# francescoalemanno/KissABC.jl

Hardware: AMD Instinct MI355X
Metric: walker proposal+cost evals/sec at N=65536 walkers, D=8 (higher is better)
Workload: dtype f64

## Files before the change

kissabc.jl_amd/csrc/ais_inst.hip:

```cpp
#define KABC_FMA_C_VGPR
#include "ais_small_kernel.hpp"

#ifndef KABC_INST_COST
#error "compile with -DKABC_INST_COST=<cost id>"
#endif

namespace kabc {

template <int D, int COST, int PC, int PK>
static void launch_half(const AisArgs& a, hipStream_t s, unsigned nchains) {
    const unsigned grid = (unsigned)((a.rows_owned + kBatch - 1) / kBatch);
    if (grid == 0) return;
    hipLaunchKernelGGL((ais_half_kernel<D, COST, PC, PK>), dim3(grid, nchains), dim3(kAisBlock), 0, s, a);
}

#ifndef KABC_INST_DLO
#define KABC_INST_DLO 1
#endif
#ifndef KABC_INST_DHI
#define KABC_INST_DHI KABC_MAX_DIM
#endif
#ifndef KABC_INST_SUFFIX
#define KABC_INST_SUFFIX
#endif
#ifndef KABC_INST_PCSEL
#define KABC_INST_PCSEL 0
#endif
template <int COST, int D, int PCX>
static AisLaunchFn pick() {
    constexpr bool is_normal = (PCX % kPriorClasses) == kPriorNormal;
    constexpr bool pc_ok = KABC_INST_PCSEL == 0 || (KABC_INST_PCSEL == 1) == is_normal;
    if constexpr (pc_ok && D >= KABC_INST_DLO && D <= KABC_INST_DHI && cost_dim_ok_c(COST, D))
        return &launch_half<D, COST, PCX % kPriorClasses, PCX / kPriorClasses + 1>;
    else return nullptr;
}

template <int COST, int PCX, int... Ds>
static AisLaunchFn row(int D, std::integer_sequence<int, Ds...>) {
    AisLaunchFn f[] = {pick<COST, Ds + 1, PCX>()...};
    return (D >= 1 && D <= (int)sizeof...(Ds)) ? f[D - 1] : nullptr;
}

template <int COST, int... PCXs>
static AisLaunchFn table(int D, int pcx, std::integer_sequence<int, PCXs...>) {
    using Dims = std::make_integer_sequence<int, KABC_MAX_DIM>;
    AisLaunchFn r = nullptr;
    ((pcx == PCXs ? (void)(r = row<COST, PCXs>(D, Dims{})) : (void)0), ...);
    return r;
}

template <int COST, int D, int PCX>
static AisSmallLaunchFn pick_small() {
    constexpr int pc = PCX % kPriorClasses;
    constexpr bool is_normal = pc == kPriorNormal;
    constexpr bool pc_ok = KABC_INST_PCSEL == 0 || (KABC_INST_PCSEL == 1) == is_normal;
    if constexpr (pc_ok && pc != kPriorSimple && D >= KABC_INST_DLO &&
                  D <= KABC_INST_DHI && cost_dim_ok_c(COST, D))
        return &launch_ais_small<D, COST, pc, PCX / kPriorClasses + 1>;
    else return nullptr;
}
template <int COST, int PCX, int... Ds>
static AisSmallLaunchFn row_small(int D, std::integer_sequence<int, Ds...>) {
    AisSmallLaunchFn f[] = {pick_small<COST, Ds + 1, PCX>()...};
    return (D >= 1 && D <= (int)sizeof...(Ds)) ? f[D - 1] : nullptr;
}
template <int COST, int... PCXs>
static AisSmallLaunchFn table_small(int D, int pcx, std::integer_sequence<int, PCXs...>) {
    using Dims = std::make_integer_sequence<int, KABC_MAX_DIM>;
    AisSmallLaunchFn r = nullptr;
    ((pcx == PCXs ? (void)(r = row_small<COST, PCXs>(D, Dims{})) : (void)0), ...);
    return r;
}

#define KABC_CAT2(a, b) a##b
#define KABC_CAT(a, b) KABC_CAT2(a, b)
AisLaunchFn KABC_CAT(KABC_CAT(find_ais_kernel_cost_, KABC_INST_COST), KABC_INST_SUFFIX)(int D, int pcx) {
    return table<KABC_INST_COST>(D, pcx, std::make_integer_sequence<int, kAisVariants>{});
}

AisSmallLaunchFn KABC_CAT(KABC_CAT(find_ais_small_kernel_cost_, KABC_INST_COST), KABC_INST_SUFFIX)(int D, int pcx) {
    return table_small<KABC_INST_COST>(D, pcx, std::make_integer_sequence<int, kAisVariants>{});
}

}
```

kissabc.jl_amd/csrc/ais_kernels.hpp:

```cpp
#pragma once

#include "kabc_device.hpp"
#ifndef __HIPCC_RTC__
#include "launcher.hpp"
#endif

namespace kabc {

struct AisArgs {
    double* x_act;
    const double* x_comp;
    double* lp;
    double* ll;
    double* trace;
    int32_t* dbg;
    DevCounters* counters;
    unsigned long long* slots;
    const double* cost_params;
    const double* cost_data;
    int64_t cost_ndata;
    int64_t row_first;
    int64_t rows_owned;
    int64_t n_comp;
    uint64_t seed;
// ... 39 lines not shown
    double eps;
    unsigned long long retry_budget;
    PriorSet prior;
    kabc_prior_t raw[KABC_MAX_DIM];
    const uint64_t* seeds;
    unsigned long long* chain_retries;
    int64_t stride_act, stride_own;
    int64_t params_stride, data_stride;
};

constexpr int kInitBlock = 64;

constexpr int kAisBlock = 256;
constexpr int kBatch = 64;
constexpr int kChunk = 3;

template <int D>
struct RecGeom {
    static constexpr int NB = (D + 2) / 2;
    static constexpr int NZ = (D + 2 > 4) ? (D + 2) : 4;
};

template <int Q>
struct SubStepIx {
    static constexpr int value = Q;
};

template <int D, int CH>
struct RecBuf {
    uint32_t mva[CH][kBatch];
// ... 327 lines not shown
        if (lane < n_active) {
            const int64_t s = (int64_t)(t - A.t0);
#pragma unroll
            for (int j = 0; j < W; ++j) aux[j][lane] = A.aux[(s * W + j) * A.rows_owned + r0 + lane];
        }
        return;
    }
    kabc_cost_rng_t rng = {A.seed, t, w_base + (uint32_t)lane, KABC_DOM_AIS_COST, 0u, 0u, nullptr,
                           logtab};
    double a[W];
    kabc_cost_prepare(COST, A.cost_params, A.cost_data, A.cost_ndata, &rng, a);
#pragma unroll
    for (int j = 0; j < W; ++j) aux[j][lane] = a[j];
}

template <int D, int COST, int PC, int PK>
__global__ void __launch_bounds__(kAisBlock) __attribute__((amdgpu_waves_per_eu(2, 2)))
ais_half_kernel(const AisArgs A0) {
    AisArgs A = A0;
    if (A0.seeds) {
        const int64_t c = (int64_t)blockIdx.y;
        A.seed = A0.seeds[c];
        A.x_act += c * A0.stride_act;
        A.x_comp += c * A0.stride_comp;
        A.lp += c * A0.stride_own;
        A.ll += c * A0.stride_own;
        if (A0.trace) A.trace += c * A0.stride_trace;
        if (A0.aux) A.aux += c * A0.stride_aux;
        A.cost_params += c * A0.params_stride;
        A.cost_data += c * A0.data_stride;
    }
    __shared__ ChunkRec<D> rec[2];
    __shared__ uint8_t listB[kChunk][kBatch];

    __shared__ PriorDev sprior[D];
    __shared__ double sbox_lo[D], sbox_hi[D];
    constexpr bool kGaussBox = PC == kPriorSimple || PC == kPriorNormal;
    __shared__ __attribute__((aligned(16))) double sgb[kGaussBox ? D : 1][8];
    __shared__ __attribute__((aligned(16))) double slogtab[KABC_MATH_TAB_WORDS];
    constexpr int kNbTabs = (PC == kPriorGeneral) ? kNbTabsGeneral : 0;
    __shared__ double snb[kNbTabs > 0 ? (kNbTabs + 1) * kNbEntries : 1];
    constexpr int kAuxW = cost_aux_c(COST);
    __shared__ double saux[2][kChunk][kAuxW > 0 ? kAuxW : 1][kBatch];
    constexpr int kPre = ais_pre_blocks(COST, D);
    __shared__ double spre[2][kChunk][kPre > 0 ? 2 * kPre : 1][kBatch];

    const int wave = __builtin_amdgcn_readfirstlane(threadIdx.x >> 6), lane = threadIdx.x & (kWave - 1);
    const int64_t r0 = (int64_t)blockIdx.x * kBatch;
    const int64_t rem = A.rows_owned - r0;
    const int n_active = rem >= kBatch ? kBatch : (int)rem;
    const uint32_t w_base = A.id_base + (uint32_t)(A.row_first + r0);
    const int nchunks = (A.nt + kChunk - 1) / kChunk;
    const bool tprobe = (KABL & 128) && A.dbg;
    unsigned long long t_begin = 0, t_bar = 0;
    if (tprobe) t_begin = __builtin_amdgcn_s_memtime();
#define KABC_TIMED_BARRIER()                                              \
    do {                                                                  \
        if (tprobe) {                                                     \
            const unsigned long long tb_ = __builtin_amdgcn_s_memtime(); \
            __syncthreads();                                              \
            t_bar += __builtin_amdgcn_s_memtime() - tb_;                  \
        } else {                                                          \
            __syncthreads();                                              \
        }                                                                 \
    } while (0)

    auto comp_row = [&](uint32_t idx) -> const double* {
        return reinterpret_cast<const double*>(reinterpret_cast<const char*>(A.x_comp) +
                                               (size_t)(idx * (uint32_t)(D * sizeof(double))));
    };
    const bool active = (wave == 0) && (lane < n_active);
    const int64_t r = r0 + lane;
    const int64_t row = A.row_first + r;
    double x[D];
    double lp = 0.0, ll = 0.0;
    unsigned int n_eval = 0, n_acc = 0;
    int err = 0;
    if (active) {
        load_row<D>(A.x_act + row * D, x);
        lp = A.lp[r];
        ll = A.ll[r];
        if (!ld_valid(PK, lp, ll)) err = 2;
    }

    static_assert(KABC_MATH_TAB_WORDS == 2 * kAisBlock, "two table words per thread");
    const double tab0 = kabc_log_tab[threadIdx.x], tab1 = kabc_log_tab[threadIdx.x + kAisBlock];
    if (threadIdx.x < D * (int)(sizeof(PriorDev) / 8))
        reinterpret_cast<double*>(sprior)[threadIdx.x] =
            reinterpret_cast<const double*>(A.prior)[threadIdx.x];
    if (threadIdx.x < D) {
        sbox_lo[threadIdx.x] = A.prior[threadIdx.x].p[0];
        sbox_hi[threadIdx.x] = A.prior[threadIdx.x].p[1];
    }
    uint32_t dmask = 0, gmask = 0;
    for (int k = 0; k < D; ++k) {
        dmask |= (A.prior[k].discrete ? 1u : 0u) << k;
        gmask |= (gaussbox_is_gauss(A.prior[k].kind) ? 1u : 0u) << k;
    }
    if constexpr (kGaussBox) {
        if (threadIdx.x < D) gaussbox_stage(sgb[threadIdx.x], A.prior[threadIdx.x]);
    }
    const GaussBoxPrior gbox = {sgb, gmask, dmask};
    constexpr bool kBoxRegs = (PC == kPriorBox) && D <= 8;
    double blo[kBoxRegs ? D : 1], bhi[kBoxRegs ? D : 1];
    const BoxPrior box = {kBoxRegs ? blo : sbox_lo, kBoxRegs ? bhi : sbox_hi, dmask, A.box_lp};

    kabc_u128_t pro01[2] = {};
    if (wave > 0 && wave - 1 < A.nt && lane < n_active) {
        const uint32_t w = w_base + (uint32_t)lane;
        const uint64_t t = A.t0 + (uint64_t)(wave - 1);
        pro01[0] = kabc_stream_block(A.seed, w, t, 0u, KABC_DOM_AIS_MOVE);
        pro01[1] = kabc_stream_block(A.seed, w, t, 1u, KABC_DOM_AIS_MOVE);
    }
    slogtab[threadIdx.x] = tab0;
    slogtab[threadIdx.x + kAisBlock] = tab1;
#ifdef KABC_MODEL_SPEC
    [[maybe_unused]] const bool nb_on = kNbTabs > 0;
#else
    [[maybe_unused]] const bool nb_on = kNbTabs > 0 && A.nt >= 8;
#endif
    if constexpr (kNbTabs > 0) {
        static_assert(kNbEntries == kAisBlock, "one table entry per thread");
        int slot = 0;
        bool has_nb = false;
        for (int k = 0; k < D; ++k) {
            if (A.prior[k].kind == KABC_PRIOR_NEGBINOMIAL) {
                has_nb = true;
                if (nb_on && slot < kNbTabs) {
                    snb[slot * kNbEntries + threadIdx.x] =
                        kabc_lgamma_t((double)threadIdx.x + A.prior[k].p[0], kabc_log_tab);
                    ++slot;
                }
            }
        }
        if (has_nb) snb[kNbLg1Block * kNbEntries + threadIdx.x] = kabc_lgamma1_tab[threadIdx.x];
    }
    KABC_TIMED_BARRIER();
    if constexpr (kNbTabs > 0) {
        if (threadIdx.x < D && sprior[threadIdx.x].kind == KABC_PRIOR_NEGBINOMIAL) {
            int slot = 0;
            for (int k = 0; k < (int)threadIdx.x; ++k)
                slot += (sprior[k].kind == KABC_PRIOR_NEGBINOMIAL) ? 1 : 0;
            sprior[threadIdx.x].p[2] = (nb_on && slot < kNbTabs) ? (double)slot : -1.0;
        }
    }
    if constexpr (kBoxRegs) {
#pragma unroll
        for (int k = 0; k < D; ++k) {
            blo[k] = sbox_lo[k];
            bhi[k] = sbox_hi[k];
        }
    }

    uint64_t seed_v = A.seed;
    asm volatile("" : "+v"(seed_v));
    constexpr bool kLate = D > kLateFrom;
    double r0a[D], r0b[D], r1a[kLate ? 1 : D], r1b[kLate ? 1 : D];
    const bool pro_rows = !(KABL & 5);
    if (wave > 0) {
        const int si = wave - 1;
        if (si < A.nt && !(KABL & 4)) {
            produce_substep<D>(A, seed_v, rec[0], si, A.t0 + (uint64_t)si, w_base, n_active, listB[si],
                               lane, slogtab, pro01, [] { __syncthreads(); });
            if constexpr (kAuxW > 0)
                prepare_cost_aux<COST, kAuxW>(A, A.t0 + (uint64_t)si, w_base, lane, saux[0][si],
                                              slogtab, r0, n_active);
            if constexpr (kPre > 0)
                produce_cost_normals<kPre>(seed_v, A.t0 + (uint64_t)si, w_base, lane, spre[0][si], slogtab);
        } else {
            __syncthreads();
        }
    } else {
        __syncthreads();
#ifndef KABC_NO_XCHUNK_PREFETCH
        if (active && pro_rows) {
            load_row<D>(comp_row(rec[0].mva[0][lane] & 0x3fffffffu), r0a);
            load_row<D>(comp_row(rec[0].bb[0][lane]), r0b);
        }
#endif
    }
    KABC_TIMED_BARRIER();

    if (wave > 0) {
#pragma unroll 1
        for (int c = 0; c < nchunks; ++c) {
            const int s0 = c * kChunk;
            const int si = wave - 1;
            const int s = s0 + kChunk + si;
            if (s < A.nt && !(KABL & 2)) {
                produce_substep<D>(A, seed_v, rec[(c + 1) & 1], si, A.t0 + (uint64_t)s, w_base, n_active,
                                   listB[si], lane, slogtab);
                if constexpr (kAuxW > 0)
                    prepare_cost_aux<COST, kAuxW>(A, A.t0 + (uint64_t)s, w_base, lane,
                                                  saux[(c + 1) & 1][si], slogtab, r0, n_active);
                if constexpr (kPre > 0)
                    produce_cost_normals<kPre>(seed_v, A.t0 + (uint64_t)s, w_base, lane,
                                               spre[(c + 1) & 1][si], slogtab);
            }
            KABC_TIMED_BARRIER();
        }
    } else {
#ifndef KABC_NO_REG_PARAMS
        constexpr int kRP = cost_reg_params(COST, D);
        double cpar[kRP > 0 ? kRP : 1];
#pragma unroll
        for (int k = 0; k < kRP; ++k) {
            cpar[k] = A.cost_params[k];
            asm volatile("" : "+v"(cpar[k]));
        }
        const double* const cparams = kRP > 0 ? cpar : A.cost_params;
#else
        const double* const cparams = A.cost_params;
#endif
        const bool dbg_on = __builtin_amdgcn_readfirstlane(A.dbg != nullptr ? 1 : 0) != 0;
#pragma unroll 1
        for (int c = 0; c < nchunks; ++c) {
            const int s0 = c * kChunk;
            if (active && !(KABL & 1)) {
                const ChunkRec<D>& R = rec[(KABL & 2) ? 0 : (c & 1)];
                const int ns = (A.nt - s0 < kChunk) ? (A.nt - s0) : kChunk;
#ifndef KABC_NO_XCHUNK_PREFETCH
                if (c > 0 || !pro_rows)
#endif
                {
                    load_row<D>(comp_row(R.mva[0][lane] & 0x3fffffffu), r0a);
                    load_row<D>(comp_row(R.bb[0][lane]), r0b);
                }
                auto substep = [&](auto SI, const double (&pa)[D], const double (&pb)[D],
                                   double (&na)[D], double (&nb)[D]) __attribute__((always_inline)) {
                    constexpr int si = decltype(SI)::value;
                    const uint64_t t = A.t0 + (uint64_t)(s0 + si);
                    constexpr int sq = si + 1 < kChunk ? si + 1 : si;
                    const uint32_t mva = R.mva[si][lane];
                    uint32_t mvan = R.mva[sq][lane], bn = R.bb[sq][lane];
                    if (si + 1 >= ns) {
                        mvan = mva;
                        bn = R.bb[si][lane];
                    }
                    const double logu = R.logu[si][lane];
                    double zs[D + 1];
#pragma unroll
                    for (int j = 0; j < D + 1; ++j) zs[j] = R.zs[si][j][lane];
                    if constexpr (!kLate) {
                        load_row<D>(comp_row(mvan & 0x3fffffffu), na);
                        load_row<D>(comp_row(bn), nb);
                    }
                    __builtin_amdgcn_sched_barrier(0);
// ... 21 lines not shown
                            const double Wk = (pa[k] - pb[k]) * gamma;
                            const double sk = kabc_fabs(pa[k] - pb[k]) + kabc_fabs(x[k] - pb[k]) +
                                              kabc_fabs(xa[k]);
                            const double Tk = kabc_div_rc(gamma * sk, 300.0, 1.0 / 300.0) * zs[1 + k];
                            y[k] = x[k] + Wk + Tk;
                        }
                    }
                    __builtin_amdgcn_sched_barrier(0);
                    if constexpr (kLate) {
                        load_row<D>(comp_row(mvan & 0x3fffffffu), na);
                        load_row<D>(comp_row(bn), nb);
                    }
                    kabc_cost_rng_t rng = {A.seed, t, w_base + (uint32_t)lane, KABC_DOM_AIS_COST, 0u,
                                           0u, nullptr, slogtab};
                    if constexpr (kAuxW > 0) {
                        rng.aux = &saux[(KABL & 2) ? 0 : (c & 1)][si][0][lane];
                        rng.aux_stride = kBatch;
                    }
                    if constexpr (kPre > 0) {
                        rng.pre = &spre[(KABL & 2) ? 0 : (c & 1)][si][0][lane];
                        rng.pre_n = (uint32_t)kPre;
                        rng.pre_stride = (uint32_t)kBatch;
                    }
                    double nlp, nll;
                    bool ev;
                    loglike<D, COST, PC>(sprior, box, gbox, PK, A.eps, A.reps, y, cparams,
                                         A.cost_data, A.cost_ndata, &rng, nlp, nll, ev, slogtab,
                                         kNbTabs > 0 ? snb : nullptr);
                    __builtin_amdgcn_sched_barrier(0);
                    n_eval += ev ? 1u : 0u;
                    const bool valid = ev && ld_valid(PK, nlp, nll);
                    const double e = -logu;
                    bool acc;
                    if (PK == KABC_POSTERIOR_KERNELIZED) {
                        const double lW = corr + (nlp + nll) - (lp + ll);
// ... 14 lines not shown
                        ll = nll;
                        n_acc += 1u;
                    }
#pragma unroll
                    for (int k = 0; k < D; ++k) asm volatile("" : "+v"(x[k]));
                    if (dbg_on) {
                        int32_t* d = A.dbg + (r * A.dbg_nt + (A.dbg_s0 + s0 + si)) * 6;
                        d[0] = (int32_t)move;
                        d[1] = acc ? 1 : 0;
                        d[2] = (int32_t)(mva & 0x3fffffffu);
                        d[3] = move >= 2u ? (int32_t)R.bb[si][lane] : -1;
                        d[4] = move == 3u ? (int32_t)R.cc[si][lane] : -1;
                        d[5] = ev ? 1 : 0;
                    }
                };
                static_assert(kChunk == 3, "the consumer spells out kChunk sub-steps");
                if constexpr (kLate) {
                    substep(SubStepIx<0>{}, r0a, r0b, r0a, r0b);
                    if (ns > 1) substep(SubStepIx<1>{}, r0a, r0b, r0a, r0b);
                    if (ns > 2) substep(SubStepIx<2>{}, r0a, r0b, r0a, r0b);
                } else {
                    substep(SubStepIx<0>{}, r0a, r0b, r1a, r1b);
                    if (ns > 1) substep(SubStepIx<1>{}, r1a, r1b, r0a, r0b);
                    if (ns > 2) substep(SubStepIx<2>{}, r0a, r0b, r1a, r1b);
                }
            }
            KABC_TIMED_BARRIER();
        }
    }

    if (tprobe && lane == 0) {
        const unsigned long long t_end = __builtin_amdgcn_s_memtime();
        int32_t* d = A.dbg + (r0 * A.nt) * 6 + 8 + wave * 2;
        d[0] = (int32_t)(t_end - t_begin);
        d[1] = (int32_t)t_bar;
    }
    if ((KABL & 64) && A.dbg && lane == 0) {
        uint32_t hw;
        asm volatile("s_getreg_b32 %0, hwreg(HW_REG_HW_ID)" : "=s"(hw));
        A.dbg[(r0 * A.nt) * 6 + wave] = (int32_t)hw;
    }
    if (wave == 0) {
        if (active) {
            store_row<D>(A.x_act + row * D, x);
            A.lp[r] = lp;
            A.ll[r] = ll;
            if (A.trace) {
                double xp[D];
#pragma unroll
                for (int k = 0; k < D; ++k)
                    xp[k] = (sprior[k].discrete && PK != KABC_POSTERIOR_COMMON)
                                ? kabc_rint(x[k]) : x[k];
                store_row<D>(A.trace + r * D, xp);
            }
        }
        const unsigned long long se = wave_total_u32(n_eval);
        const unsigned long long sa = wave_total_u32(n_acc);
        if (lane == 0) {
            unsigned long long* sl =
                A.slots + (size_t)((blockIdx.x + blockIdx.y * gridDim.x) & (kCounterSlots - 1)) * 8;
            atomicAdd(&sl[0], (unsigned long long)n_active * (unsigned long long)A.nt);
            atomicAdd(&sl[1], se);
            atomicAdd(&sl[2], sa);
        }
        if (err) atomicMax(&A.counters->error, err);
    }
}

template <int D>
__global__ void __launch_bounds__(kInitBlock) ais_init_kernel(const InitArgs A) {
    const int64_t r = (int64_t)blockIdx.x * kInitBlock + threadIdx.x;
    if (r >= A.rows_owned) return;
    const int64_t row = A.row_first + r;
    const uint32_t w = A.id_base + (uint32_t)row;
    const int64_t chain = (int64_t)blockIdx.y;
    const uint64_t seed = A.seeds ? A.seeds[chain] : A.seed;
    unsigned long long* retries = A.seeds ? A.chain_retries + chain : &A.counters->retries;
    double* x_act = A.x_act + (A.seeds ? chain * A.stride_act : 0);
    double* lp_out = A.lp + (A.seeds ? chain * A.stride_own : 0);
    double* ll_out = A.ll + (A.seeds ? chain * A.stride_own : 0);
    const double* cparams = A.cost_params + (A.seeds ? chain * A.params_stride : 0);
// ... 44 lines not shown
    lp_out[r] = lp;
    ll_out[r] = ll;
}

#ifndef __HIPCC_RTC__
using AisLaunchFn = void (*)(const AisArgs&, hipStream_t, unsigned nchains);
using AisLaunch = Launcher<AisArgs, unsigned>;
using AisInitLaunch = Launcher<InitArgs, unsigned>;
inline dim3 ais_half_geom(const AisArgs& a, unsigned nchains) {
    return dim3((unsigned)((a.rows_owned + kBatch - 1) / kBatch), nchains);
}
inline dim3 ais_init_geom(const InitArgs& a, unsigned nchains) {
    return dim3((unsigned)((a.rows_owned + kInitBlock - 1) / kInitBlock), nchains);
}
AisLaunch find_ais_kernel(int cost_id, int D, int pcx);
constexpr int kAisVariants = 3 * kPriorClasses;
struct ModelUnit;
bool launch_ais_init(int D, const InitArgs& a, hipStream_t s, unsigned nchains, ModelUnit* unit);

#endif

}
```

kissabc.jl_amd/csrc/capi_ais.hip:

```cpp
#include <chrono>
#include <condition_variable>
#include <cstdio>
#include <cstdlib>
#include <mutex>
#include <thread>
#include <type_traits>
#include <vector>

#include "ais_aux_kernels.hpp"
#include "ais_dyn_kernels.hpp"
#include "ais_dyn_small_kernel.hpp"
#include "ais_small_kernel.hpp"
#include "host_common.hpp"
#include "plugin_registry.hpp"

namespace kabc {

#define KABC_DECL_COST(id)                                                \
    AisLaunchFn find_ais_kernel_cost_##id(int D, int pc);                 \
    AisLaunchFn find_ais_kernel_cost_##id##_nrm(int D, int pc);           \
    AisLaunchFn find_ais_kernel_cost_##id##_hi(int D, int pc);            \
    AisSmallLaunchFn find_ais_small_kernel_cost_##id(int D, int pc);      \
    AisSmallLaunchFn find_ais_small_kernel_cost_##id##_nrm(int D, int pc); \
    AisSmallLaunchFn find_ais_small_kernel_cost_##id##_hi(int D, int pc);
KABC_DECL_COST(1)
KABC_DECL_COST(2)
KABC_DECL_COST(3)
KABC_DECL_COST(4)
KABC_DECL_COST(5)
KABC_DECL_COST(6)
KABC_DECL_COST(7)
KABC_DECL_COST(8)
KABC_DECL_COST(9)
KABC_DECL_COST(10)
KABC_DECL_COST(11)

// ... 12 lines not shown
        case 3: return ais_inst_pick(D, pc, find_ais_kernel_cost_3, find_ais_kernel_cost_3_nrm, find_ais_kernel_cost_3_hi);
        case 4: return ais_inst_pick(D, pc, find_ais_kernel_cost_4, find_ais_kernel_cost_4_nrm, find_ais_kernel_cost_4_hi);
        case 5: return ais_inst_pick(D, pc, find_ais_kernel_cost_5, find_ais_kernel_cost_5_nrm, find_ais_kernel_cost_5_hi);
        case 6: return ais_inst_pick(D, pc, find_ais_kernel_cost_6, find_ais_kernel_cost_6_nrm, find_ais_kernel_cost_6_hi);
        case 7: return ais_inst_pick(D, pc, find_ais_kernel_cost_7, find_ais_kernel_cost_7_nrm, find_ais_kernel_cost_7_hi);
        case 8: return ais_inst_pick(D, pc, find_ais_kernel_cost_8, find_ais_kernel_cost_8_nrm, find_ais_kernel_cost_8_hi);
        case 9: return ais_inst_pick(D, pc, find_ais_kernel_cost_9, find_ais_kernel_cost_9_nrm, find_ais_kernel_cost_9_hi);
        case 10: return ais_inst_pick(D, pc, find_ais_kernel_cost_10, find_ais_kernel_cost_10_nrm, find_ais_kernel_cost_10_hi);
        case 11: return ais_inst_pick(D, pc, find_ais_kernel_cost_11, find_ais_kernel_cost_11_nrm, find_ais_kernel_cost_11_hi);
        default: {
            const PluginKernel k = plugin_kernel(find_plugin(cost_id), kPfAis, D, pc);
            if (k.host) return AisLaunch((AisLaunchFn)k.host);
            if (k.mod) return AisLaunch(k.mod, &ais_half_geom, (unsigned)kAisBlock);
            return nullptr;
        }
    }
}

static AisSmallLaunchFn ais_small_pick(int D, int pc, AisSmallLaunchFn (*lo)(int, int), AisSmallLaunchFn (*nrm)(int, int),
                                       AisSmallLaunchFn (*hi)(int, int)) {
    if (D > kAisInstSplit) return hi(D, pc);
    return (pc % kPriorClasses) == kPriorNormal ? nrm(D, pc) : lo(D, pc);
}
AisSmallLaunch find_ais_small_kernel(int cost_id, int D, int pc) {
#define KABC_SMALL_CASE(id) \
    case id: return AisSmallLaunch(ais_small_pick(D, pc, find_ais_small_kernel_cost_##id, find_ais_small_kernel_cost_##id##_nrm, find_ais_small_kernel_cost_##id##_hi));
    switch (cost_id) {
        KABC_SMALL_CASE(1)
        KABC_SMALL_CASE(2)
        KABC_SMALL_CASE(3)
// ... 81 lines not shown
    double* d_scratch = nullptr;
    int32_t nchains = 1;
    uint64_t* d_seeds = nullptr;
    unsigned long long* d_chain_retries = nullptr;
    uint32_t id_base[2] = {};
    double* d_half[2] = {};
    bool own_halves = false;
    double* d_lp[2] = {};
    double* d_ll[2] = {};
    DevCounters* d_counters = nullptr;
    unsigned long long* d_slots = nullptr;
    PriorDev* d_prior = nullptr;
    uint64_t seed = 0, t = 0;
    int32_t rank = 0, world = 1;
    AisLaunch launch;
    int32_t pc = 0;
    bool small_ok = false;
    AisSmallLaunch small;
    int32_t small_pcx = 0;
    AisDynSmallLaunchFn dsmall = nullptr;
    AisDynSmallPlan dplan;
    double* d_strace = nullptr;
    size_t strace_cap = 0;
    ModelUnit* unit = nullptr;
    int32_t spec_state = KABC_SPEC_NONE;
    int32_t spec_variant = 0;
    int64_t launches = 0;
    int64_t spec_switch_at = -1;
    std::chrono::steady_clock::time_point spec_next_poll;
    double box_lp = 0.0;
// ... 110 lines not shown
    AisLaunch fn;
    const int pk_off = kPriorClasses * (h->posterior - 1);
    if (h->unit) {
        int st = KABC_SPEC_NONE;
        PluginKernel uk;
        if (track || unit_required(h->unit)) uk = unit_kernel(h->unit, kPfAis, h->D, h->spec_variant, &st);
        if (uk.mod) fn = AisLaunch(uk.mod, &ais_half_geom, (unsigned)kAisBlock);
        if (track) h->spec_state = st;
        if (!fn && unit_required(h->unit)) return KABC_ERR_DEVICE;
    }
    if (!fn) {
        int pc = h->pc;
        if (const char* e = std::getenv("KABC_PREBUILT_CLASS"))
            if (e[0] == 'g' && pc != kPriorBox) pc = kPriorGeneral;
        fn = find_ais_kernel(h->cost_id, h->D, pc + pk_off);
        if (!fn && h->pc == kPriorNormal)
            fn = find_ais_kernel(h->cost_id, h->D, kPriorSimple + pk_off);
    }
    if (!fn) {
        if (!get_error()[0]) set_error("no gfx950 kernel instantiated for cost id %d, D = %d", h->cost_id, h->D);
        return KABC_ERR_UNSUPPORTED;
    }
    h->launch = fn;
    return KABC_OK;
}

static kabc_status_t ais_validate(kabc_ctx_t* ctx, const kabc_model_t* m, kabc_ais_t** out, int64_t n_total,
                                  int32_t rank, int32_t world, const kabc_comm_t* comm, int32_t nchains,
                                  std::vector<kabc_prior_t>& resolved, kabc_model_t& mres) {
    if (!ctx || !m || !out || !m->prior) {
// ... 661 lines not shown
static void timing_release(kabc_ais_t* h) {
    for (hipEvent_t e : h->ev) (void)hipEventDestroy(e);
    h->ev.clear();
    for (const kabc_ais::XT& x : h->xt) xt_release(x, h->xk);
    h->xt.clear();
}

static void ais_poll_spec(kabc_ais_t* h) {
    const auto now = std::chrono::steady_clock::now();
    if (now < h->spec_next_poll) return;
    h->spec_next_poll = now + std::chrono::milliseconds(2);
    int st = KABC_SPEC_NONE;
    const PluginKernel k = unit_kernel(h->unit, h->small_ok ? kPfAisSmall : kPfAis, h->D, h->spec_variant, &st);
    if (st == KABC_SPEC_ACTIVE && k.mod) {
        if (h->small_ok) h->small = AisSmallLaunch(k.mod, &ais_small_geom, (unsigned)kAisSmallBlock);
        else h->launch = AisLaunch(k.mod, &ais_half_geom, (unsigned)kAisBlock);
        h->spec_state = KABC_SPEC_ACTIVE;
        h->spec_switch_at = h->launches;
    } else if (st == KABC_SPEC_FAILED) {
        h->spec_state = KABC_SPEC_FAILED;
    }
}

static kabc_status_t launch_half_seg(kabc_ais_t* h, int32_t half, const kabc_ais::Seg& sg,
                                     int32_t ntransitions, double* dev_trace_rows) {
    if (sg.count == 0) return KABC_OK;
    hipStream_t s = h->ctx->stream;
    if (h->spec_state == KABC_SPEC_PENDING && !h->small_ok) ais_poll_spec(h);
    if (!h->launch && !h->dyn)
        if (kabc_status_t st = ais_resolve_half(h)) return st;
    if (h->dyn && h->nchains > 1) {
        set_error("a handle of %d chains beyond %d parameters advances with kabc_ais_advance (the one-workgroup "
                  "driver); kabc_ais_half_generation drives one chain per handle there", h->nchains, KABC_MAX_DIM);
        return KABC_ERR_UNSUPPORTED;
    }
    h->launches++;
    int32_t* dbg = nullptr;
    if (h->d_dbg) {
        const int64_t off = ((half == 0 ? 0 : h->rows_owned[0]) + sg.off) * (int64_t)ntransitions * 6;
        if (off + sg.count * (int64_t)ntransitions * 6 <= h->dbg_cap) dbg = h->d_dbg + off;
    }
    const bool t_on = h->timing && (h->ev_used + 2 <= h->ev.size());
    if (t_on && h->open_count == 0) KABC_HIP_CHECK(hipEventRecord(h->ev[h->ev_used], s));
    if (h->dyn) {
        AisDynArgs a = dyn_args(h, half, sg);
        a.trace = dev_trace_rows ? dev_trace_rows + sg.off * h->D : nullptr;
        a.dbg = dbg;
        a.t0 = h->t;
        a.nt = ntransitions;
// ... 34 lines not shown
            const size_t cap = env_bytes("KABC_AUX_KIB", 1 << 10, (size_t)256 << 20);
            const size_t fit = cap / per_step;
            blk = (int32_t)(fit < 1 ? 1 : (fit > (size_t)ntransitions ? (size_t)ntransitions : fit));
            if (kabc_status_t st = grow(h, &h->d_aux, &h->aux_cap, per_step * (size_t)blk)) return st;
        }
        for (int32_t s0 = 0; s0 < ntransitions; s0 += blk) {
            const int32_t nb = ntransitions - s0 < blk ? ntransitions - s0 : blk;
            a.t0 = h->t + (uint64_t)s0;
            a.nt = nb;
            a.dbg_s0 = s0;
            a.trace = (dev_trace_rows && s0 + nb == ntransitions) ? dev_trace_rows + sg.off * h->D : nullptr;
            if (W) {
                a.aux = h->d_aux;
                a.stride_aux = enqueue_aux(h, half, sg.first, sg.count, a.t0, nb, h->d_aux);
            }
            h->launch(a, s, (unsigned)h->nchains);
        }
    }
    if (t_on && ++h->open_count >= h->timing_stride)
        if (kabc_status_t st = timing_close_pair(h)) return st;
    KABC_HIP_CHECK(hipGetLastError());
    return KABC_OK;
}

kabc_status_t kabc_ais_half_generation(kabc_ais_t* h, int32_t half, int32_t ntransitions,
                                       void* dev_trace_rows) {
    if (check_handle(h)) return KABC_ERR_INVALID_ARG;
    if (!h->initialised) {
        set_error("kabc_ais_init / kabc_ais_set_state has not been called");
        return KABC_ERR_INVALID_STATE;
    }
// ... 775 lines not shown
```

Baseline: 29.44 billion.

## Add wide 512-thread half-generation kernel with SIMD-aware producer task placement

Adds a wide variant of the AIS half-generation kernel. Each workgroup has 512 threads, with two consumer waves each owning a 64-row batch and six producer waves filling four-substep chunks. Producer tasks are handed out using the hardware SIMD id read from HW_REG_HW_ID, so that waves sharing a SIMD with a consumer take fewer tasks. The wide kernel is chosen at runtime when the cost has no aux or pre-normals, D<=8, there is a single chain, nt>=32 and rows are enough to fill the CUs. The aim is a better consumer-to-producer ratio and less per-chunk barrier overhead, at the price of more LDS per workgroup, a more complex schedule and extra instantiations.

```diff
diff --git a/kissabc.jl_amd/csrc/ais_inst.hip b/kissabc.jl_amd/csrc/ais_inst.hip
--- a/kissabc.jl_amd/csrc/ais_inst.hip
+++ b/kissabc.jl_amd/csrc/ais_inst.hip
@@ -12,6 +12,13 @@
     const unsigned grid = (unsigned)((a.rows_owned + kBatch - 1) / kBatch);
     if (grid == 0) return;
     hipLaunchKernelGGL((ais_half_kernel<D, COST, PC, PK>), dim3(grid, nchains), dim3(kAisBlock), 0, s, a);
+}
+
+template <int D, int COST, int PC, int PK, int K, int NC>
+static void launch_half_wide(const AisArgs& a, hipStream_t s, unsigned nchains) {
+    const dim3 grid = ais_wide_geom(a, nchains);
+    if (grid.x == 0) return;
+    hipLaunchKernelGGL((ais_half_wide_kernel<D, COST, PC, PK, K, NC>), grid, dim3(kWideBlock), 0, s, a);
 }
 
 #ifndef KABC_INST_DLO
@@ -35,17 +42,27 @@
     else return nullptr;
 }
 
-template <int COST, int PCX, int... Ds>
+template <int COST, int D, int PCX>
+static AisLaunchFn pick_wide() {
+    constexpr bool is_normal = (PCX % kPriorClasses) == kPriorNormal;
+    constexpr bool pc_ok = KABC_INST_PCSEL == 0 || (KABC_INST_PCSEL == 1) == is_normal;
+    if constexpr (pc_ok && D >= KABC_INST_DLO && D <= KABC_INST_DHI && cost_dim_ok_c(COST, D) &&
+                  ais_wide_ok_c(COST, D))
+        return &launch_half_wide<D, COST, PCX % kPriorClasses, PCX / kPriorClasses + 1, kWideK, kWideNC>;
+    else return nullptr;
+}
+
+template <int COST, int PCX, bool WIDE, int... Ds>
 static AisLaunchFn row(int D, std::integer_sequence<int, Ds...>) {
-    AisLaunchFn f[] = {pick<COST, Ds + 1, PCX>()...};
+    AisLaunchFn f[] = {(WIDE ? pick_wide<COST, Ds + 1, PCX>() : pick<COST, Ds + 1, PCX>())...};
     return (D >= 1 && D <= (int)sizeof...(Ds)) ? f[D - 1] : nullptr;
 }
 
-template <int COST, int... PCXs>
+template <int COST, bool WIDE, int... PCXs>
 static AisLaunchFn table(int D, int pcx, std::integer_sequence<int, PCXs...>) {
     using Dims = std::make_integer_sequence<int, KABC_MAX_DIM>;
     AisLaunchFn r = nullptr;
-    ((pcx == PCXs ? (void)(r = row<COST, PCXs>(D, Dims{})) : (void)0), ...);
+    ((pcx == PCXs ? (void)(r = row<COST, PCXs, WIDE>(D, Dims{})) : (void)0), ...);
     return r;
 }
 
@@ -75,7 +92,11 @@
 #define KABC_CAT2(a, b) a##b
 #define KABC_CAT(a, b) KABC_CAT2(a, b)
 AisLaunchFn KABC_CAT(KABC_CAT(find_ais_kernel_cost_, KABC_INST_COST), KABC_INST_SUFFIX)(int D, int pcx) {
-    return table<KABC_INST_COST>(D, pcx, std::make_integer_sequence<int, kAisVariants>{});
+    return table<KABC_INST_COST, false>(D, pcx, std::make_integer_sequence<int, kAisVariants>{});
+}
+
+AisLaunchFn KABC_CAT(KABC_CAT(find_ais_wide_kernel_cost_, KABC_INST_COST), KABC_INST_SUFFIX)(int D, int pcx) {
+    return table<KABC_INST_COST, true>(D, pcx, std::make_integer_sequence<int, kAisVariants>{});
 }
 
 AisSmallLaunchFn KABC_CAT(KABC_CAT(find_ais_small_kernel_cost_, KABC_INST_COST), KABC_INST_SUFFIX)(int D, int pcx) {
diff --git a/kissabc.jl_amd/csrc/ais_kernels.hpp b/kissabc.jl_amd/csrc/ais_kernels.hpp
--- a/kissabc.jl_amd/csrc/ais_kernels.hpp
+++ b/kissabc.jl_amd/csrc/ais_kernels.hpp
@@ -77,6 +77,18 @@
 constexpr int kAisBlock = 256;
 constexpr int kBatch = 64;
 constexpr int kChunk = 3;
+
+struct HalfGeom {
+    static constexpr bool kWide = false;
+    static constexpr int kBlock = kAisBlock, kBatches = 1, kCh = kChunk, kNC = -1;
+};
+template <int K, int NC>
+struct WideGeom {
+    static_assert(K >= 1 && K <= 8 && NC <= K, "the consumer spells out up to 8 sub-steps");
+    static constexpr bool kWide = true;
+    static constexpr int kBlock = 512, kBatches = 2, kCh = K, kNC = NC;
+};
+constexpr int kWideBlock = 512, kWideBatches = 2;
 
 template <int D>
 struct RecGeom {
@@ -434,9 +446,11 @@
     for (int j = 0; j < W; ++j) aux[j][lane] = a[j];
 }
 
-template <int D, int COST, int PC, int PK>
-__global__ void __launch_bounds__(kAisBlock) __attribute__((amdgpu_waves_per_eu(2, 2)))
-ais_half_kernel(const AisArgs A0) {
+template <int D, int COST, int PC, int PK, class G>
+__device__ __forceinline__ void ais_half_body(const AisArgs& A0) {
+    constexpr int CH = G::kCh;
+    constexpr int NBAT = G::kBatches;
+    constexpr int NPROD = G::kBlock / kWave - NBAT;
     AisArgs A = A0;
     if (A0.seeds) {
         const int64_t c = (int64_t)blockIdx.y;
@@ -450,8 +464,9 @@
         A.cost_params += c * A0.params_stride;
         A.cost_data += c * A0.data_stride;
     }
-    __shared__ ChunkRec<D> rec[2];
-    __shared__ uint8_t listB[kChunk][kBatch];
+    __shared__ RecBuf<D, CH> rec[2][NBAT];
+    __shared__ uint8_t listB[NPROD][kBatch];
+    [[maybe_unused]] __shared__ uint32_t ssimd[G::kWide ? G::kBlock / kWave : 1];
 
     __shared__ PriorDev sprior[D];
     __shared__ double sbox_lo[D], sbox_hi[D];
@@ -461,16 +476,19 @@
     constexpr int kNbTabs = (PC == kPriorGeneral) ? kNbTabsGeneral : 0;
     __shared__ double snb[kNbTabs > 0 ? (kNbTabs + 1) * kNbEntries : 1];
     constexpr int kAuxW = cost_aux_c(COST);
-    __shared__ double saux[2][kChunk][kAuxW > 0 ? kAuxW : 1][kBatch];
+    __shared__ double saux[2][NBAT][CH][kAuxW > 0 ? kAuxW : 1][kBatch];
     constexpr int kPre = ais_pre_blocks(COST, D);
-    __shared__ double spre[2][kChunk][kPre > 0 ? 2 * kPre : 1][kBatch];
+    __shared__ double spre[2][NBAT][CH][kPre > 0 ? 2 * kPre : 1][kBatch];
 
     const int wave = __builtin_amdgcn_readfirstlane(threadIdx.x >> 6), lane = threadIdx.x & (kWave - 1);
-    const int64_t r0 = (int64_t)blockIdx.x * kBatch;
+    const int bmine = (G::kWide && wave < NBAT) ? wave : 0;
+    const int64_t r0_wg = (int64_t)blockIdx.x * (NBAT * kBatch);
+    const int64_t r0 = r0_wg + bmine * kBatch;
     const int64_t rem = A.rows_owned - r0;
-    const int n_active = rem >= kBatch ? kBatch : (int)rem;
+    const int n_active = rem >= kBatch ? kBatch : (G::kWide && rem < 0) ? 0 : (int)rem;
     const uint32_t w_base = A.id_base + (uint32_t)(A.row_first + r0);
-    const int nchunks = (A.nt + kChunk - 1) / kChunk;
+    const int nchunks = (A.nt + CH - 1) / CH;
+    const bool consumer = G::kWide ? wave < NBAT : wave == 0;
     const bool tprobe = (KABL & 128) && A.dbg;
     unsigned long long t_begin = 0, t_bar = 0;
     if (tprobe) t_begin = __builtin_amdgcn_s_memtime();
@@ -489,7 +507,7 @@
         return reinterpret_cast<const double*>(reinterpret_cast<const char*>(A.x_comp) +
                                                (size_t)(idx * (uint32_t)(D * sizeof(double))));
     };
-    const bool active = (wave == 0) && (lane < n_active);
+    const bool active = consumer && (lane < n_active);
     const int64_t r = r0 + lane;
     const int64_t row = A.row_first + r;
     double x[D];
@@ -503,8 +521,11 @@
         if (!ld_valid(PK, lp, ll)) err = 2;
     }
 
-    static_assert(KABC_MATH_TAB_WORDS == 2 * kAisBlock, "two table words per thread");
-    const double tab0 = kabc_log_tab[threadIdx.x], tab1 = kabc_log_tab[threadIdx.x + kAisBlock];
+    static_assert(KABC_MATH_TAB_WORDS == 2 * kAisBlock && (G::kBlock == kAisBlock || G::kBlock == 2 * kAisBlock),
+                  "two table words per thread, or one");
+    const double tab0 = kabc_log_tab[threadIdx.x];
+    [[maybe_unused]] double tab1 = 0.0;
+    if constexpr (G::kBlock == kAisBlock) tab1 = kabc_log_tab[threadIdx.x + kAisBlock];
     if (threadIdx.x < D * (int)(sizeof(PriorDev) / 8))
         reinterpret_cast<double*>(sprior)[threadIdx.x] =
             reinterpret_cast<const double*>(A.prior)[threadIdx.x];
@@ -525,35 +546,44 @@
     double blo[kBoxRegs ? D : 1], bhi[kBoxRegs ? D : 1];
     const BoxPrior box = {kBoxRegs ? blo : sbox_lo, kBoxRegs ? bhi : sbox_hi, dmask, A.box_lp};
 
-    kabc_u128_t pro01[2] = {};
-    if (wave > 0 && wave - 1 < A.nt && lane < n_active) {
-        const uint32_t w = w_base + (uint32_t)lane;
-        const uint64_t t = A.t0 + (uint64_t)(wave - 1);
-        pro01[0] = kabc_stream_block(A.seed, w, t, 0u, KABC_DOM_AIS_MOVE);
-        pro01[1] = kabc_stream_block(A.seed, w, t, 1u, KABC_DOM_AIS_MOVE);
+    [[maybe_unused]] kabc_u128_t pro01[2] = {};
+    if constexpr (!G::kWide) {
+        if (wave > 0 && wave - 1 < A.nt && lane < n_active) {
+            const uint32_t w = w_base + (uint32_t)lane;
+            const uint64_t t = A.t0 + (uint64_t)(wave - 1);
+            pro01[0] = kabc_stream_block(A.seed, w, t, 0u, KABC_DOM_AIS_MOVE);
+            pro01[1] = kabc_stream_block(A.seed, w, t, 1u, KABC_DOM_AIS_MOVE);
+        }
     }
     slogtab[threadIdx.x] = tab0;
-    slogtab[threadIdx.x + kAisBlock] = tab1;
+    if constexpr (G::kBlock == kAisBlock) slogtab[threadIdx.x + kAisBlock] = tab1;
+    if constexpr (G::kWide) {
+        uint32_t hw;
+        asm volatile("s_getreg_b32 %0, hwreg(HW_REG_HW_ID)" : "=s"(hw));
+        if (lane == 0) ssimd[wave] = (hw >> 4) & 3u;
+    }
 #ifdef KABC_MODEL_SPEC
     [[maybe_unused]] const bool nb_on = kNbTabs > 0;
 #else
     [[maybe_unused]] const bool nb_on = kNbTabs > 0 && A.nt >= 8;
 #endif
     if constexpr (kNbTabs > 0) {
-        static_assert(kNbEntries == kAisBlock, "one table entry per thread");
+        static_assert(kNbEntries == kAisBlock, "one table entry per thread (of the first 256)");
+        const bool nb_thread = !G::kWide || threadIdx.x < (unsigned)kNbEntries;
         int slot = 0;
         bool has_nb = false;
         for (int k = 0; k < D; ++k) {
             if (A.prior[k].kind == KABC_PRIOR_NEGBINOMIAL) {
                 has_nb = true;
                 if (nb_on && slot < kNbTabs) {
-                    snb[slot * kNbEntries + threadIdx.x] =
-                        kabc_lgamma_t((double)threadIdx.x + A.prior[k].p[0], kabc_log_tab);
+                    if (nb_thread)
+                        snb[slot * kNbEntries + threadIdx.x] =
+                            kabc_lgamma_t((double)threadIdx.x + A.prior[k].p[0], kabc_log_tab);
                     ++slot;
                 }
             }
         }
-        if (has_nb) snb[kNbLg1Block * kNbEntries + threadIdx.x] = kabc_lgamma1_tab[threadIdx.x];
+        if (has_nb && nb_thread) snb[kNbLg1Block * kNbEntries + threadIdx.x] = kabc_lgamma1_tab[threadIdx.x];
     }
     KABC_TIMED_BARRIER();
     if constexpr (kNbTabs > 0) {
@@ -576,17 +606,77 @@
     asm volatile("" : "+v"(seed_v));
     constexpr bool kLate = D > kLateFrom;
     double r0a[D], r0b[D], r1a[kLate ? 1 : D], r1b[kLate ? 1 : D];
-    const bool pro_rows = !(KABL & 5);
-    if (wave > 0) {
+    const bool pro_rows = !G::kWide && !(KABL & 5);
+    [[maybe_unused]] uint32_t my_tasks = 0;
+    if constexpr (G::kWide) {
+        constexpr int NT = 2 * CH;
+        uint32_t sd = 0;
+#pragma unroll
+        for (int w = 0; w < NBAT + NPROD; ++w)
+            sd |= (uint32_t)__builtin_amdgcn_readfirstlane((int)ssimd[w]) << (4 * w);
+        const uint32_t sc0 = sd & 15u, sc1 = (sd >> 4) & 15u;
+        uint32_t cot = 0;
+        int n0 = 0, n1 = 0;
+#pragma unroll
+        for (int p = 0; p < NPROD; ++p) {
+            const uint32_t sp = (sd >> (4 * (NBAT + p))) & 15u;
+            n0 += sp == sc0 ? 1 : 0;
+            n1 += sp == sc1 ? 1 : 0;
+            cot |= (sp == sc0 || sp == sc1) ? 1u << p : 0u;
+        }
+        const bool by_place = G::kNC >= 0 && sc0 != sc1 && n0 == 1 && n1 == 1;
+        uint32_t cap = 0;
+        if (by_place) {
+            constexpr int nc = G::kNC >= 0 ? G::kNC : 0;
+            constexpr int rest = NT - 2 * nc, others = NPROD - 2;
+            int seen = 0;
+#pragma unroll
+            for (int p = 0; p < NPROD; ++p) {
+                int n = nc;
+                if (!((cot >> p) & 1u)) {
+                    n = rest / others + (seen < rest % others ? 1 : 0);
+                    ++seen;
+                }
+                cap |= (uint32_t)n << (4 * p);
+            }
+        } else {
+#pragma unroll
+            for (int p = 0; p < NPROD; ++p) cap |= (uint32_t)(NT / NPROD + (p < NT % NPROD ? 1 : 0)) << (4 * p);
+        }
+        int p = 0;
+        for (int task = 0; task < NT; ++task) {
+            while (((cap >> (4 * p)) & 15u) == 0u) p = p + 1 < NPROD ? p + 1 : 0;
+            if (p == wave - NBAT) my_tasks |= 1u << task;
+            cap -= 1u << (4 * p);
+            p = p + 1 < NPROD ? p + 1 : 0;
+        }
+    }
+    auto fill = [&](int buf, int b, int si, int s, int pw, int64_t rb, int nact, uint32_t wb,
+                    const kabc_u128_t* pre01, auto mid) __attribute__((always_inline)) {
+        produce_substep<D>(A, seed_v, rec[buf][b], si, A.t0 + (uint64_t)s, wb, nact, listB[pw], lane, slogtab,
+                           pre01, mid);
+        if constexpr (kAuxW > 0)
+            prepare_cost_aux<COST, kAuxW>(A, A.t0 + (uint64_t)s, wb, lane, saux[buf][b][si], slogtab, rb, nact);
+        if constexpr (kPre > 0)
+            produce_cost_normals<kPre>(seed_v, A.t0 + (uint64_t)s, wb, lane, spre[buf][b][si], slogtab);
+    };
+    [[maybe_unused]] auto fill_tasks = [&](int buf, int sbase) __attribute__((always_inline)) {
+#pragma unroll 1
+        for (uint32_t m = my_tasks; m != 0u; m &= m - 1u) {
+            const int task = __builtin_ctz(m);
+            const int si = task >> 1, b = task & 1;
+            const int64_t rb = r0_wg + b * kBatch, left = A.rows_owned - rb;
+            if (sbase + si < A.nt && left > 0)
+                fill(buf, b, si, sbase + si, wave - NBAT, rb, left >= kBatch ? kBatch : (int)left,
+                     A.id_base + (uint32_t)(A.row_first + rb), nullptr, NoMid());
+        }
+    };
+    if constexpr (G::kWide) {
+        if (!consumer && !(KABL & 4)) fill_tasks(0, 0);
+    } else if (wave > 0) {
         const int si = wave - 1;
         if (si < A.nt && !(KABL & 4)) {
-            produce_substep<D>(A, seed_v, rec[0], si, A.t0 + (uint64_t)si, w_base, n_active, listB[si],
-                               lane, slogtab, pro01, [] { __syncthreads(); });
-            if constexpr (kAuxW > 0)
-                prepare_cost_aux<COST, kAuxW>(A, A.t0 + (uint64_t)si, w_base, lane, saux[0][si],
-                                              slogtab, r0, n_active);
-            if constexpr (kPre > 0)
-                produce_cost_normals<kPre>(seed_v, A.t0 + (uint64_t)si, w_base, lane, spre[0][si], slogtab);
+            fill(0, 0, si, si, si, r0, n_active, w_base, pro01, [] { __syncthreads(); });
         } else {
             __syncthreads();
         }
@@ -594,28 +684,23 @@
         __syncthreads();
 #ifndef KABC_NO_XCHUNK_PREFETCH
         if (active && pro_rows) {
-            load_row<D>(comp_row(rec[0].mva[0][lane] & 0x3fffffffu), r0a);
-            load_row<D>(comp_row(rec[0].bb[0][lane]), r0b);
+            load_row<D>(comp_row(rec[0][0].mva[0][lane] & 0x3fffffffu), r0a);
+            load_row<D>(comp_row(rec[0][0].bb[0][lane]), r0b);
         }
 #endif
     }
     KABC_TIMED_BARRIER();
 
-    if (wave > 0) {
+    if (!consumer) {
 #pragma unroll 1
         for (int c = 0; c < nchunks; ++c) {
-            const int s0 = c * kChunk;
-            const int si = wave - 1;
-            const int s = s0 + kChunk + si;
-            if (s < A.nt && !(KABL & 2)) {
-                produce_substep<D>(A, seed_v, rec[(c + 1) & 1], si, A.t0 + (uint64_t)s, w_base, n_active,
-                                   listB[si], lane, slogtab);
-                if constexpr (kAuxW > 0)
-                    prepare_cost_aux<COST, kAuxW>(A, A.t0 + (uint64_t)s, w_base, lane,
-                                                  saux[(c + 1) & 1][si], slogtab, r0, n_active);
-                if constexpr (kPre > 0)
-                    produce_cost_normals<kPre>(seed_v, A.t0 + (uint64_t)s, w_base, lane,
-                                               spre[(c + 1) & 1][si], slogtab);
+            const int s0 = c * CH;
+            if constexpr (G::kWide) {
+                if (!(KABL & 2)) fill_tasks((c + 1) & 1, s0 + CH);
+            } else {
+                const int si = wave - 1;
+                const int s = s0 + CH + si;
+                if (s < A.nt && !(KABL & 2)) fill((c + 1) & 1, 0, si, s, si, r0, n_active, w_base, nullptr, NoMid());
             }
             KABC_TIMED_BARRIER();
         }
@@ -635,10 +720,10 @@
         const bool dbg_on = __builtin_amdgcn_readfirstlane(A.dbg != nullptr ? 1 : 0) != 0;
 #pragma unroll 1
         for (int c = 0; c < nchunks; ++c) {
-            const int s0 = c * kChunk;
+            const int s0 = c * CH;
             if (active && !(KABL & 1)) {
-                const ChunkRec<D>& R = rec[(KABL & 2) ? 0 : (c & 1)];
-                const int ns = (A.nt - s0 < kChunk) ? (A.nt - s0) : kChunk;
+                const RecBuf<D, CH>& R = rec[(KABL & 2) ? 0 : (c & 1)][bmine];
+                const int ns = (A.nt - s0 < CH) ? (A.nt - s0) : CH;
 #ifndef KABC_NO_XCHUNK_PREFETCH
                 if (c > 0 || !pro_rows)
 #endif
@@ -650,7 +735,7 @@
                                    double (&na)[D], double (&nb)[D]) __attribute__((always_inline)) {
                     constexpr int si = decltype(SI)::value;
                     const uint64_t t = A.t0 + (uint64_t)(s0 + si);
-                    constexpr int sq = si + 1 < kChunk ? si + 1 : si;
+                    constexpr int sq = si + 1 < CH ? si + 1 : si;
                     const uint32_t mva = R.mva[si][lane];
                     uint32_t mvan = R.mva[sq][lane], bn = R.bb[sq][lane];
                     if (si + 1 >= ns) {
@@ -702,11 +787,11 @@
                     kabc_cost_rng_t rng = {A.seed, t, w_base + (uint32_t)lane, KABC_DOM_AIS_COST, 0u,
                                            0u, nullptr, slogtab};
                     if constexpr (kAuxW > 0) {
-                        rng.aux = &saux[(KABL & 2) ? 0 : (c & 1)][si][0][lane];
+                        rng.aux = &saux[(KABL & 2) ? 0 : (c & 1)][bmine][si][0][lane];
                         rng.aux_stride = kBatch;
                     }
                     if constexpr (kPre > 0) {
-                        rng.pre = &spre[(KABL & 2) ? 0 : (c & 1)][si][0][lane];
+                        rng.pre = &spre[(KABL & 2) ? 0 : (c & 1)][bmine][si][0][lane];
                         rng.pre_n = (uint32_t)kPre;
                         rng.pre_stride = (uint32_t)kBatch;
                     }
@@ -751,15 +836,28 @@
                         d[5] = ev ? 1 : 0;
                     }
                 };
-                static_assert(kChunk == 3, "the consumer spells out kChunk sub-steps");
-                if constexpr (kLate) {
-                    substep(SubStepIx<0>{}, r0a, r0b, r0a, r0b);
-                    if (ns > 1) substep(SubStepIx<1>{}, r0a, r0b, r0a, r0b);
-                    if (ns > 2) substep(SubStepIx<2>{}, r0a, r0b, r0a, r0b);
-                } else {
-                    substep(SubStepIx<0>{}, r0a, r0b, r1a, r1b);
-                    if (ns > 1) substep(SubStepIx<1>{}, r1a, r1b, r0a, r0b);
-                    if (ns > 2) substep(SubStepIx<2>{}, r0a, r0b, r1a, r1b);
+                static_assert(CH >= 1 && CH <= 8, "the consumer spells out up to 8 sub-steps");
+                auto sub_even = [&](auto SI) __attribute__((always_inline)) {
+                    if constexpr (decltype(SI)::value < CH) {
+                        if constexpr (kLate) substep(SI, r0a, r0b, r0a, r0b);
+                        else substep(SI, r0a, r0b, r1a, r1b);
+                    }
+                };
+                auto sub_odd = [&](auto SI) __attribute__((always_inline)) {
+                    if constexpr (decltype(SI)::value < CH) {
+                        if constexpr (kLate) substep(SI, r0a, r0b, r0a, r0b);
+                        else substep(SI, r1a, r1b, r0a, r0b);
+                    }
+                };
+                sub_even(SubStepIx<0>{});
+                if (ns > 1) sub_odd(SubStepIx<1>{});
+                if (ns > 2) sub_even(SubStepIx<2>{});
+                if constexpr (CH > 3) {
+                    if (ns > 3) sub_odd(SubStepIx<3>{});
+                    if (ns > 4) sub_even(SubStepIx<4>{});
+                    if (ns > 5) sub_odd(SubStepIx<5>{});
+                    if (ns > 6) sub_even(SubStepIx<6>{});
+                    if (ns > 7) sub_odd(SubStepIx<7>{});
                 }
             }
             KABC_TIMED_BARRIER();
@@ -768,16 +866,16 @@
 
     if (tprobe && lane == 0) {
         const unsigned long long t_end = __builtin_amdgcn_s_memtime();
-        int32_t* d = A.dbg + (r0 * A.nt) * 6 + 8 + wave * 2;
+        int32_t* d = A.dbg + (r0_wg * A.nt) * 6 + 2 * (NBAT + NPROD) + wave * 2;
         d[0] = (int32_t)(t_end - t_begin);
         d[1] = (int32_t)t_bar;
     }
     if ((KABL & 64) && A.dbg && lane == 0) {
         uint32_t hw;
         asm volatile("s_getreg_b32 %0, hwreg(HW_REG_HW_ID)" : "=s"(hw));
-        A.dbg[(r0 * A.nt) * 6 + wave] = (int32_t)hw;
-    }
-    if (wave == 0) {
+        A.dbg[(r0_wg * A.nt) * 6 + wave] = (int32_t)hw;
+    }
+    if (consumer) {
         if (active) {
             store_row<D>(A.x_act + row * D, x);
             A.lp[r] = lp;
@@ -793,15 +891,28 @@
         }
         const unsigned long long se = wave_total_u32(n_eval);
         const unsigned long long sa = wave_total_u32(n_acc);
-        if (lane == 0) {
+        if (lane == 0 && (!G::kWide || n_active > 0)) {
             unsigned long long* sl =
-                A.slots + (size_t)((blockIdx.x + blockIdx.y * gridDim.x) & (kCounterSlots - 1)) * 8;
+                A.slots + (size_t)((blockIdx.x * NBAT + bmine + blockIdx.y * gridDim.x * NBAT) & (kCounterSlots - 1)) * 8;
             atomicAdd(&sl[0], (unsigned long long)n_active * (unsigned long long)A.nt);
             atomicAdd(&sl[1], se);
             atomicAdd(&sl[2], sa);
         }
         if (err) atomicMax(&A.counters->error, err);
     }
+#undef KABC_TIMED_BARRIER
+}
+
+template <int D, int COST, int PC, int PK>
+__global__ void __launch_bounds__(kAisBlock) __attribute__((amdgpu_waves_per_eu(2, 2)))
+ais_half_kernel(const AisArgs A0) {
+    ais_half_body<D, COST, PC, PK, HalfGeom>(A0);
+}
+
+template <int D, int COST, int PC, int PK, int K, int NC>
+__global__ void __launch_bounds__(kWideBlock) __attribute__((amdgpu_waves_per_eu(2, 2)))
+ais_half_wide_kernel(const AisArgs A0) {
+    ais_half_body<D, COST, PC, PK, WideGeom<K, NC>>(A0);
 }
 
 template <int D>
@@ -876,6 +987,18 @@
     return dim3((unsigned)((a.rows_owned + kInitBlock - 1) / kInitBlock), nchains);
 }
 AisLaunch find_ais_kernel(int cost_id, int D, int pcx);
+constexpr int kWideK = 4, kWideNC = 1;
+constexpr int kWideMaxDim = 8;
+constexpr bool ais_wide_ok_c(int cost, int D) {
+    const int nz = (D + 2 > 4) ? (D + 2) : 4;
+    if (D > kWideMaxDim) return false;
+    return cost < KABC_COST_USER && cost_aux_c(cost) == 0 && ais_pre_blocks(cost, D) == 0 &&
+           4 * kWideK * kBatch * (20 + 8 * nz) + (12 << 10) <= (160 << 10);
+}
+inline dim3 ais_wide_geom(const AisArgs& a, unsigned nchains) {
+    return dim3((unsigned)((a.rows_owned + kWideBatches * kBatch - 1) / (kWideBatches * kBatch)), nchains);
+}
+AisLaunch find_ais_wide_kernel(int cost_id, int D, int pcx);
 constexpr int kAisVariants = 3 * kPriorClasses;
 struct ModelUnit;
 bool launch_ais_init(int D, const InitArgs& a, hipStream_t s, unsigned nchains, ModelUnit* unit);
diff --git a/kissabc.jl_amd/csrc/capi_ais.hip b/kissabc.jl_amd/csrc/capi_ais.hip
--- a/kissabc.jl_amd/csrc/capi_ais.hip
+++ b/kissabc.jl_amd/csrc/capi_ais.hip
@@ -20,6 +20,9 @@
     AisLaunchFn find_ais_kernel_cost_##id(int D, int pc);                 \
     AisLaunchFn find_ais_kernel_cost_##id##_nrm(int D, int pc);           \
     AisLaunchFn find_ais_kernel_cost_##id##_hi(int D, int pc);            \
+    AisLaunchFn find_ais_wide_kernel_cost_##id(int D, int pc);            \
+    AisLaunchFn find_ais_wide_kernel_cost_##id##_nrm(int D, int pc);      \
+    AisLaunchFn find_ais_wide_kernel_cost_##id##_hi(int D, int pc);       \
     AisSmallLaunchFn find_ais_small_kernel_cost_##id(int D, int pc);      \
     AisSmallLaunchFn find_ais_small_kernel_cost_##id##_nrm(int D, int pc); \
     AisSmallLaunchFn find_ais_small_kernel_cost_##id##_hi(int D, int pc);
@@ -62,6 +65,17 @@
             if (k.mod) return AisLaunch(k.mod, &ais_half_geom, (unsigned)kAisBlock);
             return nullptr;
         }
+    }
+}
+
+AisLaunch find_ais_wide_kernel(int cost_id, int D, int pc) {
+    switch (cost_id) {
+#define KABC_WIDE_CASE(id) \
+    case id: return ais_inst_pick(D, pc, find_ais_wide_kernel_cost_##id, find_ais_wide_kernel_cost_##id##_nrm, find_ais_wide_kernel_cost_##id##_hi);
+        KABC_WIDE_CASE(1) KABC_WIDE_CASE(2) KABC_WIDE_CASE(3) KABC_WIDE_CASE(4) KABC_WIDE_CASE(5) KABC_WIDE_CASE(6)
+        KABC_WIDE_CASE(7) KABC_WIDE_CASE(8) KABC_WIDE_CASE(9) KABC_WIDE_CASE(10) KABC_WIDE_CASE(11)
+#undef KABC_WIDE_CASE
+        default: return nullptr;
     }
 }
 
@@ -173,6 +187,7 @@
     uint64_t seed = 0, t = 0;
     int32_t rank = 0, world = 1;
     AisLaunch launch;
+    AisLaunch launch_wide;
     int32_t pc = 0;
     bool small_ok = false;
     AisSmallLaunch small;
@@ -313,6 +328,7 @@
         if (const char* e = std::getenv("KABC_PREBUILT_CLASS"))
             if (e[0] == 'g' && pc != kPriorBox) pc = kPriorGeneral;
         fn = find_ais_kernel(h->cost_id, h->D, pc + pk_off);
+        if (fn) h->launch_wide = find_ais_wide_kernel(h->cost_id, h->D, pc + pk_off);
         if (!fn && h->pc == kPriorNormal)
             fn = find_ais_kernel(h->cost_id, h->D, kPriorSimple + pk_off);
     }
@@ -1004,12 +1020,36 @@
     const PluginKernel k = unit_kernel(h->unit, h->small_ok ? kPfAisSmall : kPfAis, h->D, h->spec_variant, &st);
     if (st == KABC_SPEC_ACTIVE && k.mod) {
         if (h->small_ok) h->small = AisSmallLaunch(k.mod, &ais_small_geom, (unsigned)kAisSmallBlock);
-        else h->launch = AisLaunch(k.mod, &ais_half_geom, (unsigned)kAisBlock);
+        else {
+            h->launch = AisLaunch(k.mod, &ais_half_geom, (unsigned)kAisBlock);
+            h->launch_wide = nullptr;
+        }
         h->spec_state = KABC_SPEC_ACTIVE;
         h->spec_switch_at = h->launches;
     } else if (st == KABC_SPEC_FAILED) {
         h->spec_state = KABC_SPEC_FAILED;
     }
+}
+
+constexpr int32_t kAisWideFrom = 32;
+static bool ais_can_wide(const kabc_ais_t* h, int64_t rows) {
+    return h->launch_wide && h->nchains == 1 && h->world == 1 && !h->comm && rows >= kWideBatches * kBatch;
+}
+static int64_t ais_wide_min_rows() {
+    static const int64_t v = [] {
+        int dev = 0, cus = 0;
+        if (hipGetDevice(&dev) != hipSuccess ||
+            hipDeviceGetAttribute(&cus, hipDeviceAttributeMultiprocessorCount, dev) != hipSuccess || cus < 1)
+            cus = 256;
+        return (int64_t)kWideBatches * kBatch * cus;
+    }();
+    return v;
+}
+static bool ais_use_wide(const kabc_ais_t* h, int64_t rows, int32_t nt) {
+    if (!ais_can_wide(h, rows)) return false;
+    const char* e = std::getenv("KABC_AIS_WIDE");
+    if (e && e[0]) return e[0] != '0';
+    return nt >= kAisWideFrom && rows >= ais_wide_min_rows();
 }
 
 static kabc_status_t launch_half_seg(kabc_ais_t* h, int32_t half, const kabc_ais::Seg& sg,
@@ -1023,6 +1063,14 @@
         set_error("a handle of %d chains beyond %d parameters advances with kabc_ais_advance (the one-workgroup "
                   "driver); kabc_ais_half_generation drives one chain per handle there", h->nchains, KABC_MAX_DIM);
         return KABC_ERR_UNSUPPORTED;
+    }
+    if (!h->dyn && !ais_can_wide(h, sg.count)) {
+        const char* e = std::getenv("KABC_AIS_WIDE");
+        if (e && e[0] == '2') {
+            set_error("KABC_AIS_WIDE=2: no wide half-generation kernel for this launch (cost id %d, D = %d, "
+                      "%lld rows, %d chains)", h->cost_id, h->D, (long long)sg.count, h->nchains);
+            return KABC_ERR_UNSUPPORTED;
+        }
     }
     h->launches++;
     int32_t* dbg = nullptr;
@@ -1087,7 +1135,7 @@
                 a.aux = h->d_aux;
                 a.stride_aux = enqueue_aux(h, half, sg.first, sg.count, a.t0, nb, h->d_aux);
             }
-            h->launch(a, s, (unsigned)h->nchains);
+            (ais_use_wide(h, sg.count, nb) ? h->launch_wide : h->launch)(a, s, (unsigned)h->nchains);
         }
     }
     if (t_on && ++h->open_count >= h->timing_stride)
```

Result: faster. 30.80 billion (median of 6 runs) (+4.6%).
